# wamuumu/query-recommendation-system

Measured on AMD Instinct MI355X. Metric: MinHash signatures/sec through the whole hot path (signatures -> LSH candidates -> pair scoring -> top-K), higher is better.
Workload: dtype u16/int32 MinHash values, uint64 keys and pairs (integer); float64 cosine

## Files before the change

### include/qrlsh.h

```cpp
#ifndef QRLSH_H
#define QRLSH_H

#include <stddef.h>
#include <stdint.h>

#ifdef __cplusplus
extern "C" {
#endif

#define QRLSH_OK 0
#define QRLSH_EINVAL (-1)
#define QRLSH_EHIP (-2)
#define QRLSH_EUNSUPPORTED (-3)
#define QRLSH_EWORKSPACE (-4)

#define QRLSH_PERM_U16 0
#define QRLSH_PERM_I32 1

#define QRLSH_SIG_I32 0
#define QRLSH_SIG_U16 1

#define QRLSH_SORT_MIX 1u
#define QRLSH_SORT_IOTA 2u
#define QRLSH_SORT_FOLD 4u
// ... 60 lines not shown
int qrlsh_unique_fill(const uint64_t *sorted, int64_t n, const void *workspace, uint64_t *out,
                      void *stream);

size_t qrlsh_row_unique_workspace_bytes(int64_t n);
int qrlsh_row_unique_count(const uint64_t *grouped, int64_t n, int32_t group_bits, int32_t id_bits,
                           uint64_t *tmp, void *workspace, size_t workspace_bytes, uint64_t *total_overflow_out,
                           void *stream);
int qrlsh_row_unique_fill(const uint64_t *tmp, int64_t n, const void *workspace, uint64_t *out, void *stream);

size_t qrlsh_region_unique_workspace_bytes(int64_t nids, int32_t group_bits);
int qrlsh_region_unique_count(const uint64_t *grouped, int64_t n, int32_t group_bits, int32_t id_bits, int64_t nids,
                              uint64_t *tmp, void *workspace, size_t workspace_bytes, uint64_t *total_overflow_out,
                              void *stream);
int qrlsh_region_unique_fill(const uint64_t *tmp, int64_t n, int32_t group_bits, int64_t nids, const void *workspace,
                             uint64_t *out, void *stream);

size_t qrlsh_pair_regions_words(int64_t n, int64_t nids, int32_t group_bits, double words_per_query);
size_t qrlsh_pair_regions_tmp_words(int64_t n, int64_t nids, int32_t group_bits, double words_per_query);
int64_t qrlsh_pair_regions_cap(int64_t n, int64_t nids, int32_t group_bits, double words_per_query);
int64_t qrlsh_pair_regions_count(int64_t n, int64_t nids, int32_t group_bits, double words_per_query);
int qrlsh_pair_regions_scatter(const uint64_t *words, int64_t n, int32_t group_bits, int64_t nids, double words_per_query,
                               uint64_t *tmp_regions, uint64_t *regions, uint32_t *counts, uint32_t *overflow_out,
                               void *stream);
int qrlsh_region_unique_count_regions(const uint64_t *regions, const uint32_t *counts, int64_t cap, int64_t n,
                                      int32_t group_bits, int32_t id_bits, int64_t nids, uint64_t *tmp, void *workspace,
                                      size_t workspace_bytes, uint64_t *total_overflow_out, void *stream);

int qrlsh_row_norms(const int32_t *sig, int64_t nq, int32_t P, int64_t *norm2_out, void *stream);
int qrlsh_verify_pairs(const void *sig, int32_t sig_dtype, int32_t P, int32_t b, const uint64_t *pairs,
                       int64_t n, uint8_t *flags_out, void *stream);
int qrlsh_score_pairs(const void *sig, int32_t sig_dtype, const int64_t *norm2, int32_t P,
                      const uint64_t *pairs, int64_t n, int32_t *milli_out, double *cos_out,
                      uint64_t *edge_out, int32_t id_bits, uint32_t *edge_dst_out, void *stream);

int qrlsh_topk_count(const uint64_t *sorted_edges, int64_t n_edges, int32_t K, int32_t id_bits,
                     void *workspace, size_t workspace_bytes, uint64_t *total_out, void *stream);
int qrlsh_topk_fill(const uint64_t *sorted_edges, const uint32_t *sorted_dst, int64_t n_edges, int32_t K,
                    int32_t id_bits, const void *workspace, int32_t *src_out, int32_t *dst_out,
                    int32_t *milli_out, void *stream);
int qrlsh_topk_fill_based(const uint64_t *sorted_edges, const uint32_t *sorted_dst, int64_t n_edges, int32_t K,
                          int32_t id_bits, int64_t src_base, const void *workspace, int32_t *src_out,
                          int32_t *dst_out, int32_t *milli_out, void *stream);

int qrlsh_score_pairs_rev(const void *sig, int32_t sig_dtype, const int64_t *norm2, int32_t P,
                          const uint64_t *pairs, int64_t n, int32_t *milli_out, uint64_t *rev_out, int32_t id_bits,
                          uint32_t *rev_dst_out, void *stream);
int qrlsh_set_score_runs(int on);
size_t qrlsh_topk_select_workspace_bytes(int64_t nq);
int qrlsh_topk_select_count(const uint64_t *pairs, int64_t n, const uint64_t *rev_sorted, const uint32_t *rev_dst,
                            int64_t nq, int32_t K, int32_t id_bits, void *workspace, size_t workspace_bytes,
                            uint64_t *total_out, void *stream);
int qrlsh_topk_select_fill(const uint64_t *pairs, const int32_t *milli, int64_t n, const uint64_t *rev_sorted,
                           const uint32_t *rev_dst, int64_t nq, int32_t K, int32_t id_bits, const void *workspace,
                           int32_t *src_out, int32_t *dst_out, int32_t *milli_out, void *stream);

int qrlsh_remap_pairs(const uint64_t *pairs, int64_t n, int64_t q0, int64_t nql, const uint64_t *need,
                      int64_t n_need, uint64_t *out, void *stream);
int qrlsh_pair_edges(const uint64_t *pairs, const int32_t *milli, int64_t n, int32_t id_bits,
                     uint64_t *fwd_out, uint64_t *rev_out, uint32_t *fwd_dst_out, uint32_t *rev_dst_out,
                     void *stream);
size_t qrlsh_idset_workspace_bytes(int64_t nids);
int qrlsh_idset_build(const uint64_t *pairs, int64_t n, int64_t q0, int64_t nql, int64_t nids, int64_t shard,
                      int32_t world, void *workspace, size_t workspace_bytes, int64_t *bounds_out, void *stream);
int qrlsh_idset_list(const void *workspace, int64_t nids, uint64_t *ids_out, void *stream);
int qrlsh_idset_remap(const uint64_t *pairs, int64_t n, int64_t q0, int64_t nql, const void *workspace,
                      int64_t nids, uint64_t *out, void *stream);
int qrlsh_gather_rows(const void *sig, int64_t row_bytes, const int64_t *norm2, const uint64_t *ids, int64_t n,
                      int64_t q0, void *rows_out, int64_t *norms_out, void *stream);
int qrlsh_score_pairs_split(const void *sig, const int64_t *norm2, int64_t split_rows, const void *sig_b,
                            const int64_t *norm2_b, int32_t sig_dtype, int32_t P, const uint64_t *pairs,
                            int64_t n, int32_t *milli_out, void *stream);
int qrlsh_edges_localize(const uint64_t *edges, const uint32_t *edge_dst, int64_t n, int32_t id_bits, int64_t q0,
                         int64_t nql, uint64_t *out, void *stream);

int qrlsh_answer_sets_count(const uint32_t *bitmaps, int64_t words_per_row, int64_t D,
                            const int32_t *qrows, int64_t nq, int32_t nfeat, int32_t *sizes_out,
                            void *stream);
// ... 81 lines not shown
```

### query-recommendation-system_amd/csrc/pairs.hip

```cpp
#include "common.h"

constexpr int PAIR_THREADS = 256;
constexpr int PAIR_IPT = 4;
constexpr int PAIR_TILE = PAIR_THREADS * PAIR_IPT;

constexpr int CMP_THREADS = 256;
constexpr int CMP_IPT = 8;
constexpr int CMP_TILE = CMP_THREADS * CMP_IPT;

constexpr int PAIR_HALO = 128;

__device__ static inline uint32_t mix_hi(uint64_t k, int hsh) { return (uint32_t)(qr_mix64(k) >> hsh); }

__device__ static inline void stage_tile(const uint64_t *__restrict__ k, int64_t nq, int64_t tile_start, int hsh,
                                         uint64_t *sk, uint32_t *sh) {
  for (int idx = threadIdx.x; idx < PAIR_HALO + PAIR_TILE; idx += PAIR_THREADS) {
    const int64_t g = tile_start - PAIR_HALO + idx;
    uint64_t key = 0;
    if (g >= 0 && g < nq) key = k[g];
    sk[idx] = key;
    sh[idx] = mix_hi(key, hsh);
  }
}

// ... 1371 lines not shown
                                        const uint64_t *rev_sorted, const uint32_t *rev_dst, int64_t nq, int32_t K,
                                        int32_t id_bits, const void *workspace, int32_t *src_out, int32_t *dst_out,
                                        int32_t *milli_out, void *stream) {
  QR_CHECK_ARG(n >= 0 && n < (1ll << 31) && nq > 0 && K > 0 && K <= SEL_MAXK && id_bits >= 1 && id_bits <= 32,
               "qrlsh_topk_select_fill: bad arguments");
  if (n == 0) return QRLSH_OK;
  QR_CHECK_ARG((pairs == nullptr) == (milli == nullptr) && rev_sorted && workspace && src_out && dst_out && milli_out,
               "qrlsh_topk_select_fill: null pointer (pairs and milli: both or neither)");
  const SelWs w = sel_ws(const_cast<void *>(workspace), nq);
  hipStream_t st = static_cast<hipStream_t>(stream);
  const uint32_t *fsp = w.fstart, *rsp = w.rstart;
  const uint64_t *offp = w.off;
  const unsigned long long *nl = reinterpret_cast<const unsigned long long *>(w.nlong);
  QR_LAUNCH("topk_select", topk_select_short_kernel, dim3((unsigned)ceil_div64(nq, 16 * SEL_QPG)), dim3(256), 0, st, pairs, milli,
            rev_sorted, rev_dst, fsp, rsp, offp, nq, K, id_bits, src_out, dst_out, milli_out);
  QR_LAUNCH("topk_select_medium", topk_select_medium_kernel, dim3(SEL_LIST_GRID), dim3(256), 0, st, pairs, milli,
            rev_sorted, rev_dst, fsp, rsp, offp, (const uint32_t *)w.medlist, nl, K, id_bits, src_out, dst_out, milli_out);
  QR_LAUNCH("topk_select_long", topk_select_long_kernel, dim3(SEL_LIST_GRID), dim3(256), 0, st, pairs, milli, rev_sorted,
            rev_dst, fsp, rsp, offp, (const uint32_t *)w.longlist, nl, K, id_bits, src_out, dst_out, milli_out,
            pairs ? 0 : 1);
  QR_LAUNCH_CHECK("qrlsh_topk_select_fill");
  return QRLSH_OK;
}
```

### query-recommendation-system_amd/csrc/sort.hip

```cpp
#include "common.h"

constexpr int SORT_THREADS = 256;
constexpr int SORT_IPT = 16;
constexpr int SORT_TILE = SORT_THREADS * SORT_IPT;
constexpr int RADIX = 256;

__device__ static inline int xcd_tile(int bid, int ntiles) {
  const int q = ntiles >> 3, r = ntiles & 7, x = bid & 7, y = bid >> 3;
  return (x < r ? x * (q + 1) : r * (q + 1) + (x - r) * q) + y;
}

enum { SM_PLAIN = 0, SM_MIX = 1, SM_FOLD = 2, SM_OWNER = 3, SM_HOST = 4 };
template <int MODE> __device__ static inline uint32_t digit_of(uint64_t key, int shift, uint32_t fold = 0) {
  if (MODE == SM_OWNER || MODE == SM_HOST) {
    const uint64_t o = MODE == SM_HOST ? qr_pair_host(key, fold) : (key >> shift) / fold;
    return o < RADIX ? (uint32_t)o : RADIX - 1;
  }
  uint64_t x = key;
  if (MODE == SM_MIX) x = qr_mix64(key);
  if (MODE == SM_FOLD) x = ((key >> 32) << fold) | (key & ((1ull << fold) - 1ull));
  return (uint32_t)(x >> shift) & (RADIX - 1);
}

template <bool SPREAD>
// ... 693 lines not shown
}

QRLSH_EXPORT size_t qrlsh_pair_regions_words(int64_t n, int64_t nids, int32_t group_bits, double words_per_query) {
  if (n <= 0 || nids <= 0 || group_bits < 0 || group_bits > 8) return 0;
  const PairRegions r = pair_regions(n, nids, group_bits, words_per_query);
  if (r.rbits > 16) return 0;
  if (!pair_regions_fit_u32(r)) return 0;
  return (size_t)r.nregions * r.cap_b;
}
QRLSH_EXPORT size_t qrlsh_pair_regions_tmp_words(int64_t n, int64_t nids, int32_t group_bits, double words_per_query) {
  if (n <= 0 || nids <= 0 || group_bits < 0 || group_bits > 8) return 0;
  const PairRegions r = pair_regions(n, nids, group_bits, words_per_query);
  return r.ra ? (size_t)r.na * r.cap_a : 0;
}
QRLSH_EXPORT int64_t qrlsh_pair_regions_cap(int64_t n, int64_t nids, int32_t group_bits, double words_per_query) {
  if (n <= 0 || nids <= 0 || group_bits < 0 || group_bits > 8) return 0;
  return (int64_t)pair_regions(n, nids, group_bits, words_per_query).cap_b;
}
QRLSH_EXPORT int64_t qrlsh_pair_regions_count(int64_t n, int64_t nids, int32_t group_bits, double words_per_query) {
  if (n <= 0 || nids <= 0 || group_bits < 0 || group_bits > 8) return 0;
  return pair_regions(n, nids, group_bits, words_per_query).nregions;
}

QRLSH_EXPORT int qrlsh_pair_regions_scatter(const uint64_t *words, int64_t n, int32_t group_bits, int64_t nids,
                                            double words_per_query, uint64_t *tmp_regions, uint64_t *regions,
                                            uint32_t *counts, uint32_t *overflow_out, void *stream) {
  QR_CHECK_ARG(n >= 0 && n < (1ll << 32) && nids > 0 && group_bits >= 0 && group_bits <= 8 && counts && overflow_out,
               "qrlsh_pair_regions_scatter: bad arguments");
  hipStream_t st = static_cast<hipStream_t>(stream);
  const PairRegions r = pair_regions(n > 0 ? n : 1, nids, group_bits, words_per_query);
  QR_CHECK_ARG(r.rbits <= 16 && r.na <= RADIX, "qrlsh_pair_regions_scatter: %d region bits", r.rbits);
  QR_CHECK_ARG(pair_regions_fit_u32(r),
               "qrlsh_pair_regions_scatter: regions reach 2^32 words (na * cap_a = %llu, 2^rb * cap_b = %llu; need both < 2^32)",
               (unsigned long long)r.na * r.cap_a, (unsigned long long)r.cap_b << r.rb);
  if (hipMemsetAsync(counts, 0, ((size_t)r.nregions + RADIX) * sizeof(uint32_t), st) != hipSuccess ||
      hipMemsetAsync(overflow_out, 0, sizeof(uint32_t), st) != hipSuccess) {
    qrlsh_set_error("qrlsh_pair_regions_scatter: hipMemsetAsync failed");
    return QRLSH_EHIP;
  }
  if (n == 0) return QRLSH_OK;
  QR_CHECK_ARG(words && regions && (r.ra == 0 || tmp_regions), "qrlsh_pair_regions_scatter: null pointer");
  const int ntiles = (int)ceil_div64(n, PG_TILE);
  const int sh = 32 + group_bits;
  if (r.ra == 0) {
    QR_LAUNCH("pair_group", (pair_group_scatter_kernel<false>), dim3(ntiles, 1), dim3(SORT_THREADS), 0, st, words, regions, n,
              ntiles, sh, (1u << r.rb) - 1u, counts, r.cap_b, overflow_out, (const uint32_t *)nullptr, 0u);
  } else {
    uint32_t *cur_a = counts + r.nregions;
    QR_LAUNCH("pair_group", (pair_group_scatter_kernel<false>), dim3(ntiles, 1), dim3(SORT_THREADS), 0, st, words, tmp_regions,
              n, ntiles, sh + r.rb, (1u << r.ra) - 1u, cur_a, r.cap_a, overflow_out, (const uint32_t *)nullptr, 0u);
    QR_LAUNCH("pair_group", (pair_group_scatter_kernel<true>), dim3((unsigned)ceil_div64(r.cap_a, PG_TILE), (unsigned)r.na),
              dim3(SORT_THREADS), 0, st, (const uint64_t *)tmp_regions, regions, (int64_t)0, 0, sh, (1u << r.rb) - 1u, counts,
              r.cap_b, overflow_out, (const uint32_t *)cur_a, r.cap_a);
  }
  QR_LAUNCH_CHECK("qrlsh_pair_regions_scatter");
  return QRLSH_OK;
}

QRLSH_EXPORT size_t qrlsh_sort_workspace_bytes(int64_t n, int32_t nbatch) {
  if (n <= 0 || nbatch <= 0) return 16;
  const int64_t ntiles = ceil_div64(n, SORT_TILE);
  return (size_t)nbatch * RADIX * (ntiles + 1) * sizeof(uint32_t);
}

template <int MIX>
static int sort_passes(uint64_t *ka, uint64_t *kb, uint32_t *va, uint32_t *vb, int64_t n, int nbatch, int bit_lo,
                       int bit_hi, bool iota, uint32_t fold, uint32_t *ghist, hipStream_t st) {
  const int ntiles = (int)ceil_div64(n, SORT_TILE);
  const dim3 grid(ntiles, nbatch), block(SORT_THREADS);
  const bool has_val = va != nullptr;
  uint32_t *rtot = ghist + (size_t)nbatch * RADIX * ntiles;
  int cur = 0;
  for (int shift = bit_lo; shift < bit_hi; shift += 8) {
    uint64_t *kin = cur ? kb : ka, *kout = cur ? ka : kb;
    uint32_t *vin = cur ? vb : va, *vout = cur ? va : vb;
    QR_LAUNCH("sort_hist", (sort_hist_kernel<MIX>), grid, block, 0, st, kin, n, ntiles, shift, ghist, (uint64_t)0, fold);
    launch_rowscan(ghist, ntiles, rtot, nbatch, st);
    if (!has_val && (MIX == SM_PLAIN || MIX == SM_FOLD))
      QR_LAUNCH("sort_scatter_k", (sort_scatter_staged_kernel<MIX>), grid, block, 0, st, kin, kout, n, ntiles, shift,
// ... 1078 lines not shown
```

### query-recommendation-system_amd/qrlsh/_lib.py

```python
import ctypes
import os

_HERE = os.path.dirname(os.path.abspath(__file__))
LIB_PATH = os.environ.get("QRLSH_LIB", os.path.join(_HERE, "libqrlsh.so"))

QRLSH_OK = 0
QRLSH_EINVAL = -1
QRLSH_EHIP = -2
QRLSH_EUNSUPPORTED = -3
QRLSH_EWORKSPACE = -4

PERM_U16 = 0
PERM_I32 = 1
SIG_I32 = 0
SIG_U16 = 1
SORT_MIX = 1
SORT_IOTA = 2
SORT_FOLD = 4
SORT_OWNER = 8
SORT_HOST = 16
SUM_PAIRWISE = 0
SUM_SEQUENTIAL = 1
RECOMMEND_MAX_K = 1024
INDEX_MAX_K = 256
# ... 20 lines not shown
    "qrlsh_pairs_fill": (ctypes.c_int, [_vp, _vp, _i64, _i32, _i32, _i32, _vp, _vp, _vp]),
    "qrlsh_bucket_workspace_bytes": (_sz, [_i64, _i32, _i32]),
    "qrlsh_bucket_pairs_count": (ctypes.c_int, [_vp, _vp, _vp, _vp, _vp, _i64, _i32, _i32, _i32, _vp, _sz, _vp, _vp]),
    "qrlsh_bucket_pairs_fill": (ctypes.c_int, [_vp, _vp, _i64, _i32, _i32, _i32, _vp, _vp, _vp]),
    "qrlsh_bucket_pairs_emit_chunked": (ctypes.c_int, [_vp, _i64, _i64, _i64, _vp, _vp, _vp, _vp, _i64, _i32, _i32, _i32, _vp, _sz, _vp, _u64, _vp, _vp]),
    "qrlsh_bucket_part_words": (_sz, [_i64, _i32, _i32]),
    "qrlsh_set_big_part_limit": (_i64, [_i64]),
    "qrlsh_set_score_runs": (_i32, [_i32]),
    "qrlsh_bucket_tmp_words": (_sz, [_i64, _i32, _i32]),
    "qrlsh_bucket_pairs_emit": (ctypes.c_int, [_vp, _vp, _vp, _vp, _vp, _i64, _i32, _i32, _i32, _vp, _sz, _vp, _u64, _vp, _vp]),
    "qrlsh_compact_workspace_bytes": (_sz, [_i64]),
    "qrlsh_row_unique_workspace_bytes": (_sz, [_i64]),
    "qrlsh_row_unique_count": (ctypes.c_int, [_vp, _i64, _i32, _i32, _vp, _vp, _sz, _vp, _vp]),
    "qrlsh_row_unique_fill": (ctypes.c_int, [_vp, _i64, _vp, _vp, _vp]),
    "qrlsh_region_unique_workspace_bytes": (_sz, [_i64, _i32]),
    "qrlsh_region_unique_count": (ctypes.c_int, [_vp, _i64, _i32, _i32, _i64, _vp, _vp, _sz, _vp, _vp]),
    "qrlsh_region_unique_fill": (ctypes.c_int, [_vp, _i64, _i32, _i64, _vp, _vp, _vp]),
    "qrlsh_region_unique_count_regions": (ctypes.c_int, [_vp, _vp, _i64, _i64, _i32, _i32, _i64, _vp, _vp, _sz, _vp, _vp]),
    "qrlsh_pair_regions_words": (_sz, [_i64, _i64, _i32, ctypes.c_double]),
    "qrlsh_pair_regions_tmp_words": (_sz, [_i64, _i64, _i32, ctypes.c_double]),
    "qrlsh_pair_regions_cap": (_i64, [_i64, _i64, _i32, ctypes.c_double]),
    "qrlsh_pair_regions_count": (_i64, [_i64, _i64, _i32, ctypes.c_double]),
    "qrlsh_pair_regions_scatter": (ctypes.c_int, [_vp, _i64, _i32, _i64, ctypes.c_double, _vp, _vp, _vp, _vp, _vp]),
    "qrlsh_unique_count": (ctypes.c_int, [_vp, _i64, _vp, _sz, _vp, _vp]),
    "qrlsh_unique_fill": (ctypes.c_int, [_vp, _i64, _vp, _vp, _vp]),
    "qrlsh_row_norms": (ctypes.c_int, [_vp, _i64, _i32, _vp, _vp]),
    "qrlsh_verify_pairs": (ctypes.c_int, [_vp, _i32, _i32, _i32, _vp, _i64, _vp, _vp]),
    "qrlsh_score_pairs": (ctypes.c_int, [_vp, _i32, _vp, _i32, _vp, _i64, _vp, _vp, _vp, _i32, _vp, _vp]),
    "qrlsh_remap_pairs": (ctypes.c_int, [_vp, _i64, _i64, _i64, _vp, _i64, _vp, _vp]),
    "qrlsh_pair_edges": (ctypes.c_int, [_vp, _vp, _i64, _i32, _vp, _vp, _vp, _vp, _vp]),
    "qrlsh_topk_count": (ctypes.c_int, [_vp, _i64, _i32, _i32, _vp, _sz, _vp, _vp]),
    "qrlsh_topk_fill": (ctypes.c_int, [_vp, _vp, _i64, _i32, _i32, _vp, _vp, _vp, _vp, _vp]),
    "qrlsh_topk_fill_based": (ctypes.c_int, [_vp, _vp, _i64, _i32, _i32, _i64, _vp, _vp, _vp, _vp, _vp]),
    "qrlsh_score_pairs_rev": (ctypes.c_int, [_vp, _i32, _vp, _i32, _vp, _i64, _vp, _vp, _i32, _vp, _vp]),
    "qrlsh_topk_select_workspace_bytes": (_sz, [_i64]),
    "qrlsh_topk_select_count": (ctypes.c_int, [_vp, _i64, _vp, _vp, _i64, _i32, _i32, _vp, _sz, _vp, _vp]),
    "qrlsh_topk_select_fill": (ctypes.c_int, [_vp, _vp, _i64, _vp, _vp, _i64, _i32, _i32, _vp, _vp, _vp, _vp, _vp]),
    "qrlsh_idset_workspace_bytes": (_sz, [_i64]),
    "qrlsh_idset_build": (ctypes.c_int, [_vp, _i64, _i64, _i64, _i64, _i64, _i32, _vp, _sz, _vp, _vp]),
    "qrlsh_idset_list": (ctypes.c_int, [_vp, _i64, _vp, _vp]),
    "qrlsh_idset_remap": (ctypes.c_int, [_vp, _i64, _i64, _i64, _vp, _i64, _vp, _vp]),
    "qrlsh_gather_rows": (ctypes.c_int, [_vp, _i64, _vp, _vp, _i64, _i64, _vp, _vp, _vp]),
    "qrlsh_score_pairs_split": (ctypes.c_int, [_vp, _vp, _i64, _vp, _vp, _i32, _i32, _vp, _i64, _vp, _vp]),
    "qrlsh_edges_localize": (ctypes.c_int, [_vp, _vp, _i64, _i32, _i64, _i64, _vp, _vp]),
    "qrlsh_answer_sets_count": (ctypes.c_int, [_vp, _i64, _i64, _vp, _i64, _i32, _vp, _vp]),
    "qrlsh_answer_sets_fill": (ctypes.c_int, [_vp, _i64, _i64, _vp, _i64, _i32, _vp, _vp, _vp]),
    "qrlsh_answer_sets_sweep": (ctypes.c_int, [_vp, _i64, _i64, _vp, _i64, _i32, _vp, _vp, _vp]),
    "qrlsh_answer_sets_compact": (ctypes.c_int, [_vp, _vp, _i64, _vp, _vp]),
    "qrlsh_predict_workspace_bytes": (_sz, [_i64, _i64, _i32]),
    "qrlsh_predict": (ctypes.c_int, [_vp, _i64, _i64, _vp, _vp, _vp, _vp, _vp, _i32, ctypes.c_double, ctypes.c_double,
                                     ctypes.c_double, _i32, _vp, _vp, _i32, _vp, _sz, _vp]),
    "qrlsh_predict_columns": (ctypes.c_int, [_vp, _i64, _i64, _vp, _vp, _vp, _i64, ctypes.c_double, ctypes.c_double,
                                             ctypes.c_double, _i32, _vp, _vp, _vp]),
    "qrlsh_index_dir_bits": (_i32, [_i64]),
    "qrlsh_index_dir_words": (_sz, [_i64, _i32]),
    "qrlsh_index_build_workspace_bytes": (_sz, [_i64, _i32]),
    "qrlsh_index_build": (ctypes.c_int, [_vp, _vp, _vp, _vp, _i64, _i32, _vp, _vp, _sz, _vp]),
    "qrlsh_index_probe_workspace_bytes": (_sz, [_i64, _i32]),
    "qrlsh_index_probe_count": (ctypes.c_int, [_vp, _vp, _i64, _i32, _i32, _vp, _i64, _vp, _sz, _vp, _vp]),
    "qrlsh_index_probe_fill": (ctypes.c_int, [_vp, _vp, _vp, _i64, _i32, _i32, _vp, _i64, _vp, _sz, _vp, _vp]),
# ... 73 lines not shown
```

### query-recommendation-system_amd/qrlsh/ops.py

```python
import ctypes

import numpy as np
import torch

from . import _lib

_vp = ctypes.c_void_p


def _stream():
    return _vp(torch.cuda.current_stream().cuda_stream)


def _ptr(t):
    if t is None:
        return None
    return _vp(t.data_ptr())


def _need(t, dtype, name, ndim=None):
    if not isinstance(t, torch.Tensor) or not t.is_cuda:
        raise TypeError("%s must be a CUDA/HIP tensor" % name)
    if t.dtype != dtype:
        raise TypeError("%s must have dtype %s, got %s" % (name, dtype, t.dtype))
# ... 673 lines not shown
    if n == 0:
        z = torch.empty((0,), dtype=torch.int32, device=dev)
        return z, z.clone(), z.clone()
    if K > SELECT_MAX_K:
        raise ValueError("topk_select handles K <= %d; use topk_edges (the sort form) beyond" % SELECT_MAX_K)
    if rdst is None:
        src_bits = id_bits if pairs is not None else local_bits_for(nq)
        rs, rd = sort_u64(rev, None, id_bits + 11, id_bits + 11 + src_bits)
    else:
        rs, rd = sort_u64(rev, rdst, 11, 11 + id_bits)
    ws = _ws(lib.qrlsh_topk_select_workspace_bytes(nq), dev)
    total = torch.zeros(1, dtype=torch.int64, device=dev)
    _lib.check(lib.qrlsh_topk_select_count(_ptr(pairs), n, _ptr(rs), _ptr(rd), int(nq), K, int(id_bits), _ptr(ws), ws.numel(),
                                           _ptr(total), _stream()))
    m = int(total.item())
    src = torch.empty((m,), dtype=torch.int32, device=dev)
    dst = torch.empty((m,), dtype=torch.int32, device=dev)
    val = torch.empty((m,), dtype=torch.int32, device=dev)
    _lib.check(lib.qrlsh_topk_select_fill(_ptr(pairs), _ptr(milli), n, _ptr(rs), _ptr(rd), int(nq), K, int(id_bits), _ptr(ws),
                                          _ptr(src), _ptr(dst), _ptr(val), _stream()))
    return src, dst, val


def remap_pairs(pairs, q0, nql, need):
    lib = _lib.load()
    _need(pairs, torch.int64, "pairs", 1)
    _need(need, torch.int64, "need", 1)
    out = torch.empty_like(pairs)
    _lib.check(lib.qrlsh_remap_pairs(_ptr(pairs), pairs.numel(), int(q0), int(nql), _ptr(need), need.numel(),
                                     _ptr(out), _stream()))
    return out


def pair_edges(pairs, milli, id_bits, wide=False):
    lib = _lib.load()
    _need(pairs, torch.int64, "pairs", 1)
    _need(milli, torch.int32, "milli", 1)
    n, dev = pairs.numel(), pairs.device
    fwd = torch.empty((n,), dtype=torch.int64, device=dev)
    rev = torch.empty((n,), dtype=torch.int64, device=dev)
    fd = torch.empty((n,), dtype=torch.int32, device=dev) if wide else None
    rd = torch.empty((n,), dtype=torch.int32, device=dev) if wide else None
    _lib.check(lib.qrlsh_pair_edges(_ptr(pairs), _ptr(milli), n, 0 if wide else int(id_bits), _ptr(fwd), _ptr(rev),
                                    _ptr(fd), _ptr(rd), _stream()))
    return ((fwd, fd), (rev, rd)) if wide else (fwd, rev)

# ... 96 lines not shown
```

### query-recommendation-system_amd/qrlsh/pipeline.py

```python
import math
import time
from dataclasses import dataclass, field

import numpy as np
import torch

from . import ops


def max_candidates(nq):
    return round(math.log(nq, 1.5))


def select_bands(P, thresh=0.2):
    for b in range(P, 0, -1):
        if P % b == 0 and b % 10 == 0:
            r = P / b
            if round((1 / b) ** (1 / r), 2) >= thresh:
                return b
    raise ValueError("no band count satisfies the reference rule for PERM=%d; pass b explicitly" % P)


@dataclass
class HotPathResult:
# ... 22 lines not shown
    stats = {}

    def tick(name, t0):
        if timings is not None:
            torch.cuda.synchronize()
            timings[name] = timings.get(name, 0.0) + (time.perf_counter() - t0)
            return time.perf_counter()
        return t0

    t0 = time.perf_counter() if timings is not None else 0.0
    if compact is None:
        compact = ops.can_compact(table)
    sig, norm2, keys = ops.minhash(offsets, rows, table, b=b, want_norm=True, compact=compact, validate=validate)
    t0 = tick("signatures", t0)
    pairs = ops.candidate_pairs(keys, r, stats, sig=sig)
    del keys
    t0 = tick("candidates", t0)
    ib = ops.id_bits_for(nq)
    if topk == "select" and (K > ops.SELECT_MAX_K or pairs.numel() >= (1 << 31)):
        topk = "sort"
    if topk == "select":
        milli, rev = ops.score_pairs_rev(sig, norm2, pairs, ib, wide=wide_ids)
        t0 = tick("scoring", t0)
        src, dst, val = ops.topk_select(pairs, milli, rev, K, ib, nq)
    else:
        milli, _, edges = ops.score_pairs(sig, norm2, pairs, edge_id_bits=ib, wide=wide_ids)
        t0 = tick("scoring", t0)
        src, dst, val = ops.topk_edges(edges, K, ib)
    tick("topk", t0)
    stats["topk"] = topk
    stats["unique_pairs"] = int(pairs.numel())
    stats["kept_edges"] = int(src.numel())
    return HotPathResult(sig, norm2, pairs, milli, src, dst, val, K, b, stats)


def sims_to_dict(src, dst, val):
    src, dst, val = ops.to_host(src), ops.to_host(dst), ops.to_host(val)
    out = {}
    if len(src) == 0:
        return out
    cut = np.flatnonzero(np.diff(src)) + 1
    starts = np.concatenate(([0], cut))
    ends = np.concatenate((cut, [len(src)]))
    for s, e in zip(starts, ends):
        out[int(src[s])] = {"indexes": dst[s:e].astype(np.int64), "values": val[s:e].astype(np.float64) / 1000.0}
    return out
```

Before: 600.3 million.

## Add region-grouped top-K selection replacing sorted select path

Adds a new top-K path that scatters reverse edges into per-group regions of 256 queries, counts per-query candidate lengths, and then does per-region top-K in shared memory. Short lists are ranked by direct comparison and long lists by a radix-histogram threshold search. Large regions spill to global memory. The goal is to avoid the global sort/select over reverse edges. It adds a host sync (info.tolist) and falls back to the old select path on overflow.

```diff
diff --git a/include/qrlsh.h b/include/qrlsh.h
--- a/include/qrlsh.h
+++ b/include/qrlsh.h
@@ -106,6 +106,9 @@
 int qrlsh_pair_regions_scatter(const uint64_t *words, int64_t n, int32_t group_bits, int64_t nids, double words_per_query,
                                uint64_t *tmp_regions, uint64_t *regions, uint32_t *counts, uint32_t *overflow_out,
                                void *stream);
+int qrlsh_pair_regions_scatter_at(const uint64_t *words, int64_t n, int32_t shift, int32_t group_bits, int64_t nids,
+                                  double words_per_query, uint64_t *tmp_regions, uint64_t *regions, uint32_t *counts,
+                                  uint32_t *overflow_out, void *stream);
 int qrlsh_region_unique_count_regions(const uint64_t *regions, const uint32_t *counts, int64_t cap, int64_t n,
                                       int32_t group_bits, int32_t id_bits, int64_t nids, uint64_t *tmp, void *workspace,
                                       size_t workspace_bytes, uint64_t *total_overflow_out, void *stream);
@@ -137,6 +140,15 @@
 int qrlsh_topk_select_fill(const uint64_t *pairs, const int32_t *milli, int64_t n, const uint64_t *rev_sorted,
                            const uint32_t *rev_dst, int64_t nq, int32_t K, int32_t id_bits, const void *workspace,
                            int32_t *src_out, int32_t *dst_out, int32_t *milli_out, void *stream);
+
+size_t qrlsh_topk_regions_workspace_bytes(int64_t nq, int32_t group_bits);
+int qrlsh_topk_regions_count(const uint64_t *pairs, int64_t n, const uint64_t *regions, const uint32_t *counts,
+                             int64_t cap, const uint32_t *overflow, int64_t nq, int32_t K, int32_t id_bits,
+                             int32_t group_bits, void *workspace, size_t workspace_bytes, uint64_t *info_out, void *stream);
+int qrlsh_topk_regions_fill(const uint64_t *pairs, const int32_t *milli, int64_t n, const uint64_t *regions,
+                            const uint32_t *counts, int64_t cap, int64_t nq, int32_t K, int32_t id_bits, int32_t group_bits,
+                            const void *workspace, uint64_t *spill, int32_t *src_out, int32_t *dst_out, int32_t *milli_out,
+                            void *stream);
 
 int qrlsh_remap_pairs(const uint64_t *pairs, int64_t n, int64_t q0, int64_t nql, const uint64_t *need,
                       int64_t n_need, uint64_t *out, void *stream);
diff --git a/query-recommendation-system_amd/csrc/pairs.hip b/query-recommendation-system_amd/csrc/pairs.hip
--- a/query-recommendation-system_amd/csrc/pairs.hip
+++ b/query-recommendation-system_amd/csrc/pairs.hip
@@ -1417,3 +1417,361 @@
   QR_LAUNCH_CHECK("qrlsh_topk_select_fill");
   return QRLSH_OK;
 }
+
+constexpr int TR_THREADS = 256;
+constexpr int TR_MAXG = 8;
+constexpr int TR_IMG = 4096;
+constexpr int TR_SHORT = 128;
+constexpr int TR_NV = 2048;
+constexpr int TR_U = 8;
+
+__device__ static inline uint32_t tr_lower(const uint64_t *__restrict__ pairs, int64_t n, uint64_t i0) {
+  int64_t lo = 0, hi = n;
+  while (lo < hi) {
+    const int64_t mid = (lo + hi) >> 1;
+    if ((pairs[mid] >> 32) >= i0) hi = mid;
+    else lo = mid + 1;
+  }
+  return (uint32_t)lo;
+}
+
+__device__ static inline uint32_t tr_scan(uint32_t v, uint32_t *wsum, uint32_t *total) {
+  const int lane = threadIdx.x & (WAVE - 1), w = threadIdx.x >> 6;
+  uint32_t inc = v;
+#pragma unroll
+  for (int d = 1; d < WAVE; d <<= 1) {
+    const uint32_t o = __shfl_up(inc, d, WAVE);
+    if (lane >= d) inc += o;
+  }
+  if (lane == WAVE - 1) wsum[w] = inc;
+  __syncthreads();
+  uint32_t ex = inc - v, tot = 0;
+#pragma unroll
+  for (int k = 0; k < TR_THREADS / WAVE; ++k) {
+    if (k < w) ex += wsum[k];
+    tot += wsum[k];
+  }
+  *total = tot;
+  __syncthreads();
+  return ex;
+}
+
+__global__ __launch_bounds__(TR_THREADS) void topk_region_count_kernel(
+    const uint64_t *__restrict__ pairs, int64_t n, const uint64_t *__restrict__ regions,
+    const uint32_t *__restrict__ counts, uint32_t cap, const uint32_t *__restrict__ overflow, int64_t nq, int K,
+    int id_bits, int g, uint32_t *__restrict__ fbound, uint64_t *__restrict__ rtotal, uint64_t *__restrict__ spoff,
+    uint32_t *__restrict__ qlen, unsigned long long *__restrict__ info) {
+  __shared__ uint32_t lcnt[1 << TR_MAXG];
+  __shared__ uint32_t sf[2];
+  __shared__ uint32_t wsum[TR_THREADS / WAVE];
+  const int t = threadIdx.x;
+  const uint32_t G = 1u << g, r = blockIdx.x;
+  const int64_t q0 = (int64_t)r << g;
+  if (t < (int)G) lcnt[t] = 0;
+  if (t == 0) sf[0] = tr_lower(pairs, n, (uint64_t)q0);
+  if (t == WAVE) sf[1] = tr_lower(pairs, n, (uint64_t)(q0 + G));
+  if (r == 0 && t == 0) info[1] = *overflow;
+  __syncthreads();
+  const uint32_t f0 = sf[0], f1 = sf[1];
+  for (uint32_t x0 = f0; x0 < f1; x0 += TR_THREADS * TR_U) {
+    uint32_t qv[TR_U];
+#pragma unroll
+    for (int u = 0; u < TR_U; ++u) {
+      const uint32_t x = x0 + u * TR_THREADS + t;
+      qv[u] = x < f1 ? (uint32_t)(pairs[x] >> 32) & (G - 1) : 0xFFFFFFFFu;
+    }
+#pragma unroll
+    for (int u = 0; u < TR_U; ++u)
+      if (qv[u] != 0xFFFFFFFFu) atomicAdd(&lcnt[qv[u]], 1u);
+  }
+  const uint32_t rc = min(counts[r], cap);
+  const uint64_t *reg = regions + (size_t)r * cap;
+  const int sh = id_bits + 11;
+  for (uint32_t k0 = 0; k0 < rc; k0 += TR_THREADS * TR_U) {
+    uint32_t qv[TR_U];
+#pragma unroll
+    for (int u = 0; u < TR_U; ++u) {
+      const uint32_t k = k0 + u * TR_THREADS + t;
+      qv[u] = k < rc ? (uint32_t)(reg[k] >> sh) & (G - 1) : 0xFFFFFFFFu;
+    }
+#pragma unroll
+    for (int u = 0; u < TR_U; ++u)
+      if (qv[u] != 0xFFFFFFFFu) atomicAdd(&lcnt[qv[u]], 1u);
+  }
+  __syncthreads();
+  uint32_t c = 0;
+  if (t < (int)G && q0 + t < nq) {
+    const uint32_t len = lcnt[t];
+    qlen[q0 + t] = len;
+    c = len < (uint32_t)K ? len : (uint32_t)K;
+  }
+  uint32_t tot;
+  tr_scan(c, wsum, &tot);
+  if (t == 0) {
+    fbound[r] = f0;
+    rtotal[r] = tot;
+    if (r == gridDim.x - 1) {
+      fbound[r + 1] = f1;
+      rtotal[r + 1] = 0;
+    }
+    const uint32_t e = (f1 - f0) + rc;
+    if (e > (uint32_t)TR_IMG) {
+      spoff[r] = __hip_atomic_fetch_add(&info[3], (unsigned long long)e, __ATOMIC_RELAXED, __HIP_MEMORY_SCOPE_AGENT);
+      __hip_atomic_fetch_add(&info[2], 1ull, __ATOMIC_RELAXED, __HIP_MEMORY_SCOPE_AGENT);
+    }
+  }
+}
+
+struct TrShared {
+  uint32_t lst[(1 << TR_MAXG) + 1], ost[1 << TR_MAXG], len[1 << TR_MAXG], cur[1 << TR_MAXG];
+  uint32_t hist[TR_NV];
+  uint64_t keep[SEL_MAXK];
+  uint32_t wsum[TR_THREADS / WAVE];
+  uint32_t d, below, hd, nk;
+};
+
+__device__ static inline void tr_fill_region(uint64_t *img, TrShared &s, const uint64_t *__restrict__ pairs,
+                                             const int32_t *__restrict__ milli, const uint64_t *__restrict__ reg,
+                                             uint32_t f0, uint32_t f1, uint32_t rc, int64_t q0, uint32_t G, int64_t nq,
+                                             int K, int id_bits, const uint32_t *__restrict__ qlen, uint64_t obase,
+                                             int32_t *__restrict__ src_out, int32_t *__restrict__ dst_out,
+                                             int32_t *__restrict__ milli_out) {
+  const int t = threadIdx.x;
+  const uint32_t len = (t < (int)G && q0 + t < nq) ? qlen[q0 + t] : 0u;
+  uint32_t e, m;
+  const uint32_t ls = tr_scan(len, s.wsum, &e);
+  const uint32_t os = tr_scan(len < (uint32_t)K ? len : (uint32_t)K, s.wsum, &m);
+  if (t < (int)G) {
+    s.lst[t] = ls;
+    s.ost[t] = os;
+    s.len[t] = len;
+    s.cur[t] = ls;
+  }
+  if (t == 0) s.lst[G] = e;
+  __syncthreads();
+  for (uint32_t x0 = f0; x0 < f1; x0 += TR_THREADS * TR_U) {
+    uint64_t w[TR_U];
+    int32_t v[TR_U];
+#pragma unroll
+    for (int u = 0; u < TR_U; ++u) {
+      const uint32_t x = x0 + u * TR_THREADS + t;
+      w[u] = x < f1 ? pairs[x] : 0ull;
+      v[u] = x < f1 ? milli[x] : 0;
+    }
+#pragma unroll
+    for (int u = 0; u < TR_U; ++u) {
+      if (x0 + u * TR_THREADS + t < f1) {
+        const uint32_t p = atomicAdd(&s.cur[(uint32_t)(w[u] >> 32) & (G - 1)], 1u);
+        if (p < e) img[p] = (uint64_t)(uint32_t)(1000 - v[u]) << 32 | (uint32_t)w[u];
+      }
+    }
+  }
+  const int sh = id_bits + 11;
+  const uint64_t idm = (1ull << id_bits) - 1ull;
+  for (uint32_t k0 = 0; k0 < rc; k0 += TR_THREADS * TR_U) {
+    uint64_t w[TR_U];
+#pragma unroll
+    for (int u = 0; u < TR_U; ++u) {
+      const uint32_t k = k0 + u * TR_THREADS + t;
+      w[u] = k < rc ? reg[k] : 0ull;
+    }
+#pragma unroll
+    for (int u = 0; u < TR_U; ++u) {
+      if (k0 + u * TR_THREADS + t < rc) {
+        const uint32_t p = atomicAdd(&s.cur[(uint32_t)(w[u] >> sh) & (G - 1)], 1u);
+        if (p < e) img[p] = ((w[u] >> id_bits) & 0x7FFull) << 32 | (w[u] & idm);
+      }
+    }
+  }
+  __syncthreads();
+  for (uint32_t p = t; p < e; p += TR_THREADS) {
+    uint32_t lo = 0, hi = G;
+    while (hi - lo > 1) {
+      const uint32_t mid = (lo + hi) >> 1;
+      if (s.lst[mid] <= p) lo = mid;
+      else hi = mid;
+    }
+    const uint32_t L = s.len[lo];
+    if (L > (uint32_t)TR_SHORT) continue;
+    const uint32_t b = s.lst[lo];
+    const uint64_t mine = img[p];
+    uint32_t rank = 0;
+    for (uint32_t x = 0; x < L; ++x) rank += img[b + x] < mine;
+    if (rank < (uint32_t)K) {
+      const uint64_t o = obase + s.ost[lo] + rank;
+      src_out[o] = (int32_t)(q0 + lo);
+      dst_out[o] = (int32_t)(uint32_t)mine;
+      milli_out[o] = 1000 - (int32_t)(uint32_t)(mine >> 32);
+    }
+  }
+  for (uint32_t q = 0; q < G; ++q) {
+    const uint32_t L = s.len[q];
+    if (L <= (uint32_t)TR_SHORT) continue;
+    const uint32_t b = s.lst[q];
+    uint64_t cut = ~0ull;
+    if (L > (uint32_t)K) {
+      uint32_t need = (uint32_t)K;
+      uint64_t prefix = 0;
+      int shp = 43;
+      for (int l = 0; l < 4; ++l) {
+        const int shl = l == 0 ? 32 : l == 1 ? 22 : l == 2 ? 11 : 0;
+        const uint32_t dm = (1u << (shp - shl)) - 1u;
+        for (int v = t; v < TR_NV; v += TR_THREADS) s.hist[v] = 0;
+        __syncthreads();
+        for (uint32_t x = t; x < L; x += TR_THREADS) {
+          const uint64_t k = img[b + x];
+          if (l == 0 || (k >> shp) == prefix) atomicAdd(&s.hist[(uint32_t)(k >> shl) & dm], 1u);
+        }
+        __syncthreads();
+        constexpr int PER = TR_NV / TR_THREADS;
+        uint32_t h8 = 0;
+#pragma unroll
+        for (int v = 0; v < PER; ++v) h8 += s.hist[t * PER + v];
+        uint32_t tot;
+        const uint32_t ex = tr_scan(h8, s.wsum, &tot);
+        if (ex < need && need <= ex + h8) {
+          uint32_t run = ex;
+          for (int v = 0; v < PER; ++v) {
+            const uint32_t h = s.hist[t * PER + v];
+            if (run + h >= need) {
+              s.d = t * PER + v;
+              s.below = run;
+              s.hd = h;
+              break;
+            }
+            run += h;
+          }
+        }
+        __syncthreads();
+        const uint32_t d = s.d, hd = s.hd;
+        need -= s.below;
+        prefix = (prefix << (shp - shl)) | d;
+        shp = shl;
+        if (hd == need) break;
+      }
+      cut = (prefix << shp) | ((1ull << shp) - 1ull);
+    }
+    if (t == 0) s.nk = 0;
+    __syncthreads();
+    for (uint32_t x = t; x < L; x += TR_THREADS) {
+      const uint64_t k = img[b + x];
+      if (k <= cut) {
+        const uint32_t a = atomicAdd(&s.nk, 1u);
+        if (a < (uint32_t)SEL_MAXK) s.keep[a] = k;
+      }
+    }
+    __syncthreads();
+    const uint32_t nk = min(s.nk, (uint32_t)SEL_MAXK);
+    for (uint32_t a = t; a < nk; a += TR_THREADS) {
+      const uint64_t k = s.keep[a];
+      uint32_t rank = 0;
+      for (uint32_t c = 0; c < nk; ++c) rank += s.keep[c] < k;
+      const uint64_t o = obase + s.ost[q] + rank;
+      src_out[o] = (int32_t)(q0 + q);
+      dst_out[o] = (int32_t)(uint32_t)k;
+      milli_out[o] = 1000 - (int32_t)(uint32_t)(k >> 32);
+    }
+    __syncthreads();
+  }
+}
+
+__global__ __launch_bounds__(TR_THREADS) void topk_region_fill_kernel(
+    const uint64_t *__restrict__ pairs, const int32_t *__restrict__ milli, const uint64_t *__restrict__ regions,
+    const uint32_t *__restrict__ counts, uint32_t cap, int64_t nq, int K, int id_bits, int g,
+    const uint32_t *__restrict__ fbound, const uint64_t *__restrict__ roff, const uint64_t *__restrict__ spoff,
+    const uint32_t *__restrict__ qlen, uint64_t *__restrict__ spill, int32_t *__restrict__ src_out,
+    int32_t *__restrict__ dst_out, int32_t *__restrict__ milli_out) {
+  __shared__ uint64_t img[TR_IMG];
+  __shared__ TrShared s;
+  const uint32_t r = blockIdx.x, G = 1u << g;
+  const uint32_t f0 = fbound[r], f1 = fbound[r + 1], rc = min(counts[r], cap);
+  const uint32_t e = (f1 - f0) + rc;
+  if (e == 0) return;
+  const uint64_t *reg = regions + (size_t)r * cap;
+  if (e <= (uint32_t)TR_IMG)
+    tr_fill_region(img, s, pairs, milli, reg, f0, f1, rc, (int64_t)r << g, G, nq, K, id_bits, qlen, roff[r], src_out,
+                   dst_out, milli_out);
+  else
+    tr_fill_region(spill + spoff[r], s, pairs, milli, reg, f0, f1, rc, (int64_t)r << g, G, nq, K, id_bits, qlen, roff[r],
+                   src_out, dst_out, milli_out);
+}
+
+struct TrWs {
+  uint32_t *fbound, *qlen;
+  uint64_t *roff, *spoff, *sums;
+  size_t bytes;
+};
+static TrWs tr_ws(void *workspace, int64_t nq, int g) {
+  TrWs w;
+  const int64_t nr = (nq + (1ll << g) - 1) >> g;
+  char *p = static_cast<char *>(workspace);
+  size_t o = 0;
+  w.fbound = reinterpret_cast<uint32_t *>(p + o);
+  o += ((size_t)(nr + 1) * 4 + 15) & ~(size_t)15;
+  w.roff = reinterpret_cast<uint64_t *>(p + o);
+  o += (size_t)(nr + 2) * 8;
+  w.spoff = reinterpret_cast<uint64_t *>(p + o);
+  o += (size_t)(nr + 2) * 8;
+  w.qlen = reinterpret_cast<uint32_t *>(p + o);
+  o += ((size_t)(nr << g) * 4 + 15) & ~(size_t)15;
+  w.sums = reinterpret_cast<uint64_t *>(p + o);
+  o += (size_t)(ceil_div64(nr + 1, SCANL_CHUNK) + 2) * 8;
+  w.bytes = o;
+  return w;
+}
+
+QRLSH_EXPORT size_t qrlsh_topk_regions_workspace_bytes(int64_t nq, int32_t group_bits) {
+  if (nq <= 0 || group_bits < 0 || group_bits > TR_MAXG) return 64;
+  return tr_ws(nullptr, nq, group_bits).bytes;
+}
+
+QRLSH_EXPORT int qrlsh_topk_regions_count(const uint64_t *pairs, int64_t n, const uint64_t *regions,
+                                          const uint32_t *counts, int64_t cap, const uint32_t *overflow, int64_t nq,
+                                          int32_t K, int32_t id_bits, int32_t group_bits, void *workspace,
+                                          size_t workspace_bytes, uint64_t *info_out, void *stream) {
+  QR_CHECK_ARG(n > 0 && n < (1ll << 31) && nq > 0 && K > 0 && K <= SEL_MAXK && id_bits >= 1 && id_bits <= 26 &&
+                   group_bits >= 0 && group_bits <= TR_MAXG && ((nq + (1ll << group_bits) - 1) >> group_bits) <= 65536 &&
+                   ((nq - 1) >> id_bits) == 0 && cap > 0 && cap < (1ll << 32),
+               "qrlsh_topk_regions_count: bad arguments (n=%lld nq=%lld K=%d id_bits=%d group_bits=%d)", (long long)n,
+               (long long)nq, K, id_bits, group_bits);
+  QR_CHECK_ARG(pairs && regions && counts && overflow && workspace && info_out, "qrlsh_topk_regions_count: null pointer");
+  if (workspace_bytes < qrlsh_topk_regions_workspace_bytes(nq, group_bits)) {
+    qrlsh_set_error("qrlsh_topk_regions_count: workspace %zu < %zu bytes", workspace_bytes,
+                    qrlsh_topk_regions_workspace_bytes(nq, group_bits));
+    return QRLSH_EWORKSPACE;
+  }
+  hipStream_t st = static_cast<hipStream_t>(stream);
+  const TrWs w = tr_ws(workspace, nq, group_bits);
+  const int64_t nr = (nq + (1ll << group_bits) - 1) >> group_bits;
+  if (hipMemsetAsync(info_out, 0, 4 * sizeof(uint64_t), st) != hipSuccess) {
+    qrlsh_set_error("qrlsh_topk_regions_count: hipMemsetAsync failed");
+    return QRLSH_EHIP;
+  }
+  QR_LAUNCH("topk_region_count", topk_region_count_kernel, dim3((unsigned)nr), dim3(TR_THREADS), 0, st, pairs, n,
+            regions, counts, (uint32_t)cap, overflow, nq, K, id_bits, group_bits, w.fbound, w.roff, w.spoff, w.qlen,
+            reinterpret_cast<unsigned long long *>(info_out));
+  qr_scan_u64(w.roff, nr + 1, info_out, w.sums, st);
+  QR_LAUNCH_CHECK("qrlsh_topk_regions_count");
+  return QRLSH_OK;
+}
+
+QRLSH_EXPORT int qrlsh_topk_regions_fill(const uint64_t *pairs, const int32_t *milli, int64_t n, const uint64_t *regions,
+                                         const uint32_t *counts, int64_t cap, int64_t nq, int32_t K, int32_t id_bits,
+                                         int32_t group_bits, const void *workspace, uint64_t *spill, int32_t *src_out,
+                                         int32_t *dst_out, int32_t *milli_out, void *stream) {
+  QR_CHECK_ARG(n > 0 && n < (1ll << 31) && nq > 0 && K > 0 && K <= SEL_MAXK && id_bits >= 1 && id_bits <= 26 &&
+                   group_bits >= 0 && group_bits <= TR_MAXG && ((nq + (1ll << group_bits) - 1) >> group_bits) <= 65536 &&
+                   cap > 0 && cap < (1ll << 32),
+               "qrlsh_topk_regions_fill: bad arguments");
+  QR_CHECK_ARG(pairs && milli && regions && counts && workspace && spill && src_out && dst_out && milli_out,
+               "qrlsh_topk_regions_fill: null pointer");
+  hipStream_t st = static_cast<hipStream_t>(stream);
+  const TrWs w = tr_ws(const_cast<void *>(workspace), nq, group_bits);
+  const int64_t nr = (nq + (1ll << group_bits) - 1) >> group_bits;
+  QR_LAUNCH("topk_region_fill", topk_region_fill_kernel, dim3((unsigned)nr), dim3(TR_THREADS), 0, st, pairs, milli,
+            regions, counts, (uint32_t)cap, nq, K, id_bits, group_bits, (const uint32_t *)w.fbound,
+            (const uint64_t *)w.roff, (const uint64_t *)w.spoff, (const uint32_t *)w.qlen, spill, src_out, dst_out,
+            milli_out);
+  QR_LAUNCH_CHECK("qrlsh_topk_regions_fill");
+  return QRLSH_OK;
+}
diff --git a/query-recommendation-system_amd/csrc/sort.hip b/query-recommendation-system_amd/csrc/sort.hip
--- a/query-recommendation-system_amd/csrc/sort.hip
+++ b/query-recommendation-system_amd/csrc/sort.hip
@@ -739,39 +739,54 @@
   return pair_regions(n, nids, group_bits, words_per_query).nregions;
 }
 
+static int pair_regions_scatter(const char *fn, const char *label, const uint64_t *words, int64_t n, int shift,
+                                int32_t group_bits, int64_t nids, double words_per_query, uint64_t *tmp_regions,
+                                uint64_t *regions, uint32_t *counts, uint32_t *overflow_out, void *stream) {
+  QR_CHECK_ARG(n >= 0 && n < (1ll << 32) && nids > 0 && group_bits >= 0 && group_bits <= 8 && shift >= 0 &&
+                   shift + group_bits < 64 && counts && overflow_out,
+               "%s: bad arguments", fn);
+  hipStream_t st = static_cast<hipStream_t>(stream);
+  const PairRegions r = pair_regions(n > 0 ? n : 1, nids, group_bits, words_per_query);
+  QR_CHECK_ARG(r.rbits <= 16 && r.na <= RADIX, "%s: %d region bits", fn, r.rbits);
+  QR_CHECK_ARG(pair_regions_fit_u32(r),
+               "%s: regions reach 2^32 words (na * cap_a = %llu, 2^rb * cap_b = %llu; need both < 2^32)", fn,
+               (unsigned long long)r.na * r.cap_a, (unsigned long long)r.cap_b << r.rb);
+  if (hipMemsetAsync(counts, 0, ((size_t)r.nregions + RADIX) * sizeof(uint32_t), st) != hipSuccess ||
+      hipMemsetAsync(overflow_out, 0, sizeof(uint32_t), st) != hipSuccess) {
+    qrlsh_set_error("%s: hipMemsetAsync failed", fn);
+    return QRLSH_EHIP;
+  }
+  if (n == 0) return QRLSH_OK;
+  QR_CHECK_ARG(words && regions && (r.ra == 0 || tmp_regions), "%s: null pointer", fn);
+  const int ntiles = (int)ceil_div64(n, PG_TILE);
+  const int sh = shift + group_bits;
+  if (r.ra == 0) {
+    QR_LAUNCH(label, (pair_group_scatter_kernel<false>), dim3(ntiles, 1), dim3(SORT_THREADS), 0, st, words, regions, n,
+              ntiles, sh, (1u << r.rb) - 1u, counts, r.cap_b, overflow_out, (const uint32_t *)nullptr, 0u);
+  } else {
+    uint32_t *cur_a = counts + r.nregions;
+    QR_LAUNCH(label, (pair_group_scatter_kernel<false>), dim3(ntiles, 1), dim3(SORT_THREADS), 0, st, words, tmp_regions,
+              n, ntiles, sh + r.rb, (1u << r.ra) - 1u, cur_a, r.cap_a, overflow_out, (const uint32_t *)nullptr, 0u);
+    QR_LAUNCH(label, (pair_group_scatter_kernel<true>), dim3((unsigned)ceil_div64(r.cap_a, PG_TILE), (unsigned)r.na),
+              dim3(SORT_THREADS), 0, st, (const uint64_t *)tmp_regions, regions, (int64_t)0, 0, sh, (1u << r.rb) - 1u, counts,
+              r.cap_b, overflow_out, (const uint32_t *)cur_a, r.cap_a);
+  }
+  QR_LAUNCH_CHECK(fn);
+  return QRLSH_OK;
+}
+
 QRLSH_EXPORT int qrlsh_pair_regions_scatter(const uint64_t *words, int64_t n, int32_t group_bits, int64_t nids,
                                             double words_per_query, uint64_t *tmp_regions, uint64_t *regions,
                                             uint32_t *counts, uint32_t *overflow_out, void *stream) {
-  QR_CHECK_ARG(n >= 0 && n < (1ll << 32) && nids > 0 && group_bits >= 0 && group_bits <= 8 && counts && overflow_out,
-               "qrlsh_pair_regions_scatter: bad arguments");
-  hipStream_t st = static_cast<hipStream_t>(stream);
-  const PairRegions r = pair_regions(n > 0 ? n : 1, nids, group_bits, words_per_query);
-  QR_CHECK_ARG(r.rbits <= 16 && r.na <= RADIX, "qrlsh_pair_regions_scatter: %d region bits", r.rbits);
-  QR_CHECK_ARG(pair_regions_fit_u32(r),
-               "qrlsh_pair_regions_scatter: regions reach 2^32 words (na * cap_a = %llu, 2^rb * cap_b = %llu; need both < 2^32)",
-               (unsigned long long)r.na * r.cap_a, (unsigned long long)r.cap_b << r.rb);
-  if (hipMemsetAsync(counts, 0, ((size_t)r.nregions + RADIX) * sizeof(uint32_t), st) != hipSuccess ||
-      hipMemsetAsync(overflow_out, 0, sizeof(uint32_t), st) != hipSuccess) {
-    qrlsh_set_error("qrlsh_pair_regions_scatter: hipMemsetAsync failed");
-    return QRLSH_EHIP;
-  }
-  if (n == 0) return QRLSH_OK;
-  QR_CHECK_ARG(words && regions && (r.ra == 0 || tmp_regions), "qrlsh_pair_regions_scatter: null pointer");
-  const int ntiles = (int)ceil_div64(n, PG_TILE);
-  const int sh = 32 + group_bits;
-  if (r.ra == 0) {
-    QR_LAUNCH("pair_group", (pair_group_scatter_kernel<false>), dim3(ntiles, 1), dim3(SORT_THREADS), 0, st, words, regions, n,
-              ntiles, sh, (1u << r.rb) - 1u, counts, r.cap_b, overflow_out, (const uint32_t *)nullptr, 0u);
-  } else {
-    uint32_t *cur_a = counts + r.nregions;
-    QR_LAUNCH("pair_group", (pair_group_scatter_kernel<false>), dim3(ntiles, 1), dim3(SORT_THREADS), 0, st, words, tmp_regions,
-              n, ntiles, sh + r.rb, (1u << r.ra) - 1u, cur_a, r.cap_a, overflow_out, (const uint32_t *)nullptr, 0u);
-    QR_LAUNCH("pair_group", (pair_group_scatter_kernel<true>), dim3((unsigned)ceil_div64(r.cap_a, PG_TILE), (unsigned)r.na),
-              dim3(SORT_THREADS), 0, st, (const uint64_t *)tmp_regions, regions, (int64_t)0, 0, sh, (1u << r.rb) - 1u, counts,
-              r.cap_b, overflow_out, (const uint32_t *)cur_a, r.cap_a);
-  }
-  QR_LAUNCH_CHECK("qrlsh_pair_regions_scatter");
-  return QRLSH_OK;
+  return pair_regions_scatter("qrlsh_pair_regions_scatter", "pair_group", words, n, 32, group_bits, nids,
+                              words_per_query, tmp_regions, regions, counts, overflow_out, stream);
+}
+
+QRLSH_EXPORT int qrlsh_pair_regions_scatter_at(const uint64_t *words, int64_t n, int32_t shift, int32_t group_bits,
+                                               int64_t nids, double words_per_query, uint64_t *tmp_regions,
+                                               uint64_t *regions, uint32_t *counts, uint32_t *overflow_out, void *stream) {
+  return pair_regions_scatter("qrlsh_pair_regions_scatter_at", "topk_group", words, n, shift, group_bits, nids,
+                              words_per_query, tmp_regions, regions, counts, overflow_out, stream);
 }
 
 QRLSH_EXPORT size_t qrlsh_sort_workspace_bytes(int64_t n, int32_t nbatch) {
diff --git a/query-recommendation-system_amd/qrlsh/_lib.py b/query-recommendation-system_amd/qrlsh/_lib.py
--- a/query-recommendation-system_amd/qrlsh/_lib.py
+++ b/query-recommendation-system_amd/qrlsh/_lib.py
@@ -66,6 +66,7 @@
     "qrlsh_pair_regions_cap": (_i64, [_i64, _i64, _i32, ctypes.c_double]),
     "qrlsh_pair_regions_count": (_i64, [_i64, _i64, _i32, ctypes.c_double]),
     "qrlsh_pair_regions_scatter": (ctypes.c_int, [_vp, _i64, _i32, _i64, ctypes.c_double, _vp, _vp, _vp, _vp, _vp]),
+    "qrlsh_pair_regions_scatter_at": (ctypes.c_int, [_vp, _i64, _i32, _i32, _i64, ctypes.c_double, _vp, _vp, _vp, _vp, _vp]),
     "qrlsh_unique_count": (ctypes.c_int, [_vp, _i64, _vp, _sz, _vp, _vp]),
     "qrlsh_unique_fill": (ctypes.c_int, [_vp, _i64, _vp, _vp, _vp]),
     "qrlsh_row_norms": (ctypes.c_int, [_vp, _i64, _i32, _vp, _vp]),
@@ -80,6 +81,10 @@
     "qrlsh_topk_select_workspace_bytes": (_sz, [_i64]),
     "qrlsh_topk_select_count": (ctypes.c_int, [_vp, _i64, _vp, _vp, _i64, _i32, _i32, _vp, _sz, _vp, _vp]),
     "qrlsh_topk_select_fill": (ctypes.c_int, [_vp, _vp, _i64, _vp, _vp, _i64, _i32, _i32, _vp, _vp, _vp, _vp, _vp]),
+    "qrlsh_topk_regions_workspace_bytes": (_sz, [_i64, _i32]),
+    "qrlsh_topk_regions_count": (ctypes.c_int, [_vp, _i64, _vp, _vp, _i64, _vp, _i64, _i32, _i32, _i32, _vp, _sz, _vp, _vp]),
+    "qrlsh_topk_regions_fill": (ctypes.c_int, [_vp, _vp, _i64, _vp, _vp, _i64, _i64, _i32, _i32, _i32, _vp, _vp, _vp, _vp, _vp,
+                                                _vp]),
     "qrlsh_idset_workspace_bytes": (_sz, [_i64]),
     "qrlsh_idset_build": (ctypes.c_int, [_vp, _i64, _i64, _i64, _i64, _i64, _i32, _vp, _sz, _vp, _vp]),
     "qrlsh_idset_list": (ctypes.c_int, [_vp, _i64, _vp, _vp]),
diff --git a/query-recommendation-system_amd/qrlsh/ops.py b/query-recommendation-system_amd/qrlsh/ops.py
--- a/query-recommendation-system_amd/qrlsh/ops.py
+++ b/query-recommendation-system_amd/qrlsh/ops.py
@@ -719,6 +719,58 @@
     return src, dst, val
 
 
+TOPK_REGION_GROUP_BITS = 8
+
+
+def topk_regions(pairs, milli, rev, K, id_bits, nq, stats=None):
+    lib = _lib.load()
+    if isinstance(rev, tuple) or pairs is None:
+        return None
+    n = rev.numel()
+    if n == 0 or K > SELECT_MAX_K or id_bits > 26 or n >= (1 << 31):
+        return None
+    g = min(TOPK_REGION_GROUP_BITS, id_bits)
+    if (nq + (1 << g) - 1) >> g > 65536:
+        return None
+    dev = rev.device
+    words = lib.qrlsh_pair_regions_words(n, nq, g, 0.0)
+    twords = lib.qrlsh_pair_regions_tmp_words(n, nq, g, 0.0)
+    if words == 0 or (words + twords) * 8 > REGION_SCATTER_MAX_BYTES:
+        return None
+    cap = lib.qrlsh_pair_regions_cap(n, nq, g, 0.0)
+    nreg = lib.qrlsh_pair_regions_count(n, nq, g, 0.0)
+    try:
+        regions = torch.empty((words,), dtype=torch.int64, device=dev)
+        tmpr = torch.empty((twords,), dtype=torch.int64, device=dev) if twords else None
+    except torch.cuda.OutOfMemoryError:
+        regions = tmpr = None
+        torch.cuda.empty_cache()
+        return None
+    counts = torch.empty((nreg + 256,), dtype=torch.int32, device=dev)
+    ovf = torch.empty((1,), dtype=torch.int32, device=dev)
+    _lib.check(lib.qrlsh_pair_regions_scatter_at(_ptr(rev), n, int(id_bits) + 11, g, int(nq), 0.0, _ptr(tmpr),
+                                                 _ptr(regions), _ptr(counts), _ptr(ovf), _stream()))
+    del tmpr
+    ws = _ws(lib.qrlsh_topk_regions_workspace_bytes(nq, g), dev)
+    info = torch.empty((4,), dtype=torch.int64, device=dev)
+    _lib.check(lib.qrlsh_topk_regions_count(_ptr(pairs), n, _ptr(regions), _ptr(counts), cap, _ptr(ovf), int(nq), K,
+                                            int(id_bits), g, _ptr(ws), ws.numel(), _ptr(info), _stream()))
+    m, overflow, nbig, nspill = info.tolist()
+    if overflow:
+        return None
+    if stats is not None:
+        stats["topk_big_regions"] = int(nbig)
+    spill = torch.empty((max(nspill, 1),), dtype=torch.int64, device=dev)
+    src = torch.empty((m,), dtype=torch.int32, device=dev)
+    dst = torch.empty((m,), dtype=torch.int32, device=dev)
+    val = torch.empty((m,), dtype=torch.int32, device=dev)
+    if m:
+        _lib.check(lib.qrlsh_topk_regions_fill(_ptr(pairs), _ptr(milli), n, _ptr(regions), _ptr(counts), cap, int(nq), K,
+                                               int(id_bits), g, _ptr(ws), _ptr(spill), _ptr(src), _ptr(dst), _ptr(val),
+                                               _stream()))
+    return src, dst, val
+
+
 def remap_pairs(pairs, q0, nql, need):
     lib = _lib.load()
     _need(pairs, torch.int64, "pairs", 1)
diff --git a/query-recommendation-system_amd/qrlsh/pipeline.py b/query-recommendation-system_amd/qrlsh/pipeline.py
--- a/query-recommendation-system_amd/qrlsh/pipeline.py
+++ b/query-recommendation-system_amd/qrlsh/pipeline.py
@@ -68,7 +68,9 @@
     if topk == "select":
         milli, rev = ops.score_pairs_rev(sig, norm2, pairs, ib, wide=wide_ids)
         t0 = tick("scoring", t0)
-        src, dst, val = ops.topk_select(pairs, milli, rev, K, ib, nq)
+        got = ops.topk_regions(pairs, milli, rev, K, ib, nq, stats)
+        stats["topk_form"] = "regions" if got is not None else "select"
+        src, dst, val = got if got is not None else ops.topk_select(pairs, milli, rev, K, ib, nq)
     else:
         milli, _, edges = ops.score_pairs(sig, norm2, pairs, edge_id_bits=ib, wide=wide_ids)
         t0 = tick("scoring", t0)
```

Measured after the change: 572.2 million, median of 2. -4.7%, worse.
